# GTEC-UDC/roskfpos

Measured on AMD Instinct MI355X. Metric: EKF predict+update steps/s at 65536 tags x 8 anchors; RMS pos err vs CPU ref, higher is better.
Workload: dtype f64 arithmetic; f64 state and covariance, f32/int32 measurements in HBM (KFPOS_STORE_MIXED)

## Files before the change

__graft_entry__.py:

```python
from __future__ import annotations

import os
import shutil
import subprocess
import sys

ROOT = os.path.dirname(os.path.abspath(__file__))
CSRC = os.path.join(ROOT, "roskfpos_amd", "csrc")
HIP_LIB = os.path.join(CSRC, "libkfpos_hip.so")
ADAPTOR_DEMO = os.path.join(CSRC, "kfpos_replay")


def _stale(target, sources):
    if not os.path.exists(target):
        return True
    mt = os.path.getmtime(target)
    return any(os.path.getmtime(s) > mt for s in sources if os.path.exists(s))


def build(force: bool = False) -> None:
    jobs = str(min(8, os.cpu_count() or 1))
    res = subprocess.run(["make", "-s", "-j", jobs, "-C", CSRC] + (["-B"] if force else []) + ["all"],
                         capture_output=True, text=True)
    if res.returncode != 0:
        sys.stderr.write(res.stdout + res.stderr)
        raise subprocess.CalledProcessError(res.returncode, res.args)
    res = subprocess.run(["make", "-s", "-C", CSRC, "check"], capture_output=True, text=True)
    if res.returncode != 0:
        sys.stderr.write(res.stdout + res.stderr)
        if os.path.exists(HIP_LIB):
            os.remove(HIP_LIB)
        raise RuntimeError("a build-time performance rule is broken (scratch inside a loop / a kernel lost its second "
                           "wavefront per SIMD / the 9-state epoch loop waits for a memory operation just issued / a trip of its gain "
                           "iteration touches memory or branches too often): " + (res.stdout + res.stderr).strip())
    subprocess.check_call(["make", "-s", "-C", os.path.join(ROOT, "oracle")] + (["-B"] if force else []))
    import glob
    core_headers = sorted(glob.glob(os.path.join(CSRC, "kfpos_core*.h"))) + [os.path.join(CSRC, "kfpos_p48.h")]
    emu_dir = os.path.join(ROOT, "tests", "emu")
    emu_so = os.path.join(emu_dir, "libkfpos_emu.so")
    if force or _stale(emu_so, [os.path.join(emu_dir, "kfpos_emu.cpp")] + core_headers):
        subprocess.check_call(["g++", "-O2", "-std=c++17", "-fPIC", "-shared", "-Wno-unknown-pragmas",
                               "-o", emu_so, os.path.join(emu_dir, "kfpos_emu.cpp")])
    fake_dir = os.path.join(ROOT, "tests", "fake_rccl")
    fake_so = os.path.join(fake_dir, "libfake_rccl.so")
    if force or _stale(fake_so, [os.path.join(fake_dir, "fake_rccl.cpp")]):
        subprocess.check_call([shutil.which("hipcc") or "/opt/rocm/bin/hipcc", "-O2", "-std=c++17", "-shared", "-fPIC",
                               "-o", fake_so, os.path.join(fake_dir, "fake_rccl.cpp"), "-lrt"])
    if ROOT not in sys.path:
        sys.path.insert(0, ROOT)
    import roskfpos_amd
    from roskfpos_amd import capi
    capi.load()


def smoke() -> None:
    if ROOT not in sys.path:
        sys.path.insert(0, ROOT)
    sys.path.insert(0, os.path.join(ROOT, "oracle"))
    import numpy as np
    from roskfpos_amd import capi
    from roskfpos_amd.synth import Workload
    import oracle_py

    T, A, S = 256, 8, 12
    w = Workload(T, A)
    for model in (capi.MODEL_TOA, capi.MODEL_TOA_IMU):
        bank = capi.KfposBank(model, T, w.anchors, init_pos=w.init_positions())
        orc = oracle_py.OracleBank(model, T, w.anchors, init_pos=w.init_positions(), n_threads=4)
        err, cov = w.err_est(), w.accel_cov()
        for s in range(S):
            r, a, dt = w.ranges_mm(s), w.accel(s), w.dt_of(s)
            if model == capi.MODEL_TOA_IMU:
                bank.step_toa_imu(r, err, a, cov, dt)
                orc.step_imu(a, cov, 0.0)
                orc.step_toa(r, err, dt)
            else:
                bank.step_toa(r, err, dt)
                orc.step_toa(r, err, dt)
        x, _, _ = bank.get_state()
        xo, _ = orc.get_state()
        rms = float(np.sqrt(((x[:, :3] - xo[:, :3]) ** 2).sum(1).mean()))
        print(f"smoke model={model}: RMS position difference vs oracle = {rms:.3e} m")
        assert rms <= 1e-6, rms
        bank.close()


if __name__ == "__main__":
    build()
    if len(sys.argv) > 1 and sys.argv[1] == "smoke":
        smoke()
```

roskfpos_amd/csrc/kfpos_core_imu9.h:

```cpp
#ifndef KFPOS_CORE_IMU9_H
#define KFPOS_CORE_IMU9_H

namespace kfpos {

constexpr double INFO_FORM_MIN_PIVOT = 1e-7;

struct Tag9 {
    double pos[3], vel[3];
    Cov<9, true> P;
};
struct Imu {
    bool has;
    double acc[3];
    double *ci;
    int ci_stride;
    KFPOS_HD double Wi(int k) const { return ci[(6 + k) * ci_stride]; }
};

KFPOS_FN void imu_whitener(const double s[9], double *ci, int ci_stride) {
    double c00, c11, c22, i00, i11, i22;
    kf_sqrt_rsqrt(s[0], c00, i00);
    const double c10 = s[3] * i00, c20 = s[6] * i00;
    kf_sqrt_rsqrt(s[4] - c10 * c10, c11, i11);
    const double c21 = (s[7] - c20 * c10) * i11;
    kf_sqrt_rsqrt(s[8] - c20 * c20 - c21 * c21, c22, i22);
    const double i10 = -c10 * i00 * i11;
    const double i21 = -c21 * i11 * i22;
    const double i20 = -(c20 * i00 + c21 * i10) * i22;
    ci[0] = i00; ci[ci_stride] = i10; ci[2 * ci_stride] = i20; ci[3 * ci_stride] = i11; ci[4 * ci_stride] = i21;
    ci[5 * ci_stride] = i22;
    double *wi = ci + 6 * ci_stride;
    wi[0] = i00 * i00 + i10 * i10 + i20 * i20;
    wi[ci_stride] = i10 * i11 + i20 * i21;
    wi[2 * ci_stride] = i20 * i22;
    wi[3 * ci_stride] = i11 * i11 + i21 * i21;
    wi[4 * ci_stride] = i21 * i22;
    wi[5 * ci_stride] = i22 * i22;
}

KFPOS_FN void predict9(Cov<9, true> &P, double t, double jolt) {
    const double c = t * t / 2;
    KFPOS_UNROLL
    for (int i = 0; i < 3; ++i) {
        KFPOS_UNROLL
        for (int j = i; j < 3; ++j) {
            const double xpp = P(i, j) + t * P(3 + i, j) + c * P(6 + i, j);
            const double xpv = P(i, 3 + j) + t * P(3 + i, 3 + j) + c * P(6 + i, 3 + j);
            const double xpa = P(i, 6 + j) + t * P(3 + i, 6 + j) + c * P(6 + i, 6 + j);
            P(i, j) = xpp + t * xpv + c * xpa;
        }
    }
    KFPOS_UNROLL
    for (int i = 0; i < 3; ++i) {
        KFPOS_UNROLL
        for (int j = 0; j < 3; ++j) {
            const double xpv = P(i, 3 + j) + t * P(3 + i, 3 + j) + c * P(6 + i, 3 + j);
            const double xpa = P(i, 6 + j) + t * P(3 + i, 6 + j) + c * P(6 + i, 6 + j);
            P(i, 3 + j) = xpv + t * xpa;
        }
    }
    KFPOS_UNROLL
    for (int i = 0; i < 3; ++i) {
        KFPOS_UNROLL
        for (int j = 0; j < 3; ++j) P(i, 6 + j) = P(i, 6 + j) + t * P(3 + i, 6 + j) + c * P(6 + i, 6 + j);
    }
    KFPOS_UNROLL
    for (int i = 0; i < 3; ++i) {
        KFPOS_UNROLL
        for (int j = i; j < 3; ++j) {
            const double xvv = P(3 + i, 3 + j) + t * P(6 + i, 3 + j);
            const double xva = P(3 + i, 6 + j) + t * P(6 + i, 6 + j);
            P(3 + i, 3 + j) = xvv + t * xva;
        }
    }
    KFPOS_UNROLL
    for (int i = 0; i < 3; ++i) {
        KFPOS_UNROLL
        for (int j = 0; j < 3; ++j) P(3 + i, 6 + j) = P(3 + i, 6 + j) + t * P(6 + i, 6 + j);
    }
    const double u[3] = {(t * t * t) / 6, (t * t) / 2, t};
    KFPOS_UNROLL
    for (int k = 0; k < 3; ++k) {
        KFPOS_UNROLL
        for (int a = 0; a < 3; ++a) {
            KFPOS_UNROLL
            for (int b = a; b < 3; ++b) P(k + 3 * a, k + 3 * b) += jolt * u[a] * u[b];
        }
    }
}

KFPOS_HD constexpr int e9(int k) { return k < 3 ? k : k + 3; }

struct Factor9 {
    double lr[6], ilr[3];
    double la[6];
};
KFPOS_FN void factor9(const double mr[6], const double acc[3], const Imu &imu, Factor9 &f) {
    chol3_psd(mr, f.lr, f.ilr);
    if (imu.has) {
        const int cs = imu.ci_stride;
        f.la[0] = acc[0] * imu.ci[0]; f.la[1] = acc[0] * imu.ci[cs]; f.la[2] = acc[0] * imu.ci[2 * cs];
        f.la[3] = acc[1] * imu.ci[3 * cs]; f.la[4] = acc[1] * imu.ci[4 * cs];
        f.la[5] = acc[2] * imu.ci[5 * cs];
    } else {
        KFPOS_UNROLL
        for (int k = 0; k < 6; ++k) f.la[k] = 0.0;
    }
}
KFPOS_FN double L9(const Factor9 &f, int k, int l) {
    if (k < 3 && l < 3) {
        if (k < l) return 0.0;
        return f.lr[l == 0 ? k : (l == 1 ? 2 + k : 5)];
    }
    if (k >= 3 && l >= 3) {
        const int i = k - 3, j = l - 3;
        if (i > j) return 0.0;
        return f.la[i == 0 ? j : (i == 1 ? 2 + j : 5)];
    }
    return 0.0;
}

struct Iekf9Out {
    double w[6];
    double mrlast[6], dlast[3];
    double cost;
    int gain_iters, ml_iters;
    uint32_t flags;
};

template <class SC>
KFPOS_FN void iekf9_weights(const double xhat[9], SC &sc, const Params &pr, bool has_ranging, int n_used,
                            Iekf9Out &o) {
    o.flags = (has_ranging && n_used < 4) ? ST_FEW_RANGES : 0u;
    o.ml_iters = 0;
    if (has_ranging) {
        double pml[3] = {xhat[0], xhat[1], xhat[2]}, e_ml;
        set_weights_ml(sc, pr, 0ull);
        o.ml_iters = ml_estimate(pml, sc, pr, 0ull, n_used, e_ml);
        if (ml_covariance_throws(sc, pr, 0ull, n_used, e_ml)) o.flags |= ST_UPDATE_SKIPPED;
        set_weights_iekf(sc, pr, e_ml, 0ull);
    }
}

template <bool DIAG, bool RANGING, class SC>
KFPOS_FN void iekf9(const double xhat[9], const Cov<9, true> &P, SC &sc, const Params &pr,
                    const Imu &imu, int max_steps, double tol, Iekf9Out &o) {
    double p[3] = {xhat[0], xhat[1], xhat[2]}, acc[3] = {xhat[6], xhat[7], xhat[8]};
    double ve[6] = {0, 0, 0, 0, 0, 0};
    double wl[6] = {0, 0, 0, 0, 0, 0};
    double qd = 0.0, cost = 1e20;
    const bool pivot = RANGING && illconditioned(sc, pr, P);
    KFPOS_UNROLL
    for (int k = 0; k < 6; ++k) o.mrlast[k] = 0.0;
    o.dlast[0] = o.dlast[1] = o.dlast[2] = 0.0;
    o.gain_iters = 0;
    for (int iter = 0; iter < max_steps; ++iter) {
        double c = qd, m0 = 0, m1 = 0, m2 = 0, m3 = 0, m4 = 0, m5 = 0, u0 = 0, u1 = 0, u2 = 0;
        if constexpr (RANGING) {
            for_anchors<SC>(pr, [&](int a) {
                const double dx = p[0] - pr.anchors[3 * a], dy = p[1] - pr.anchors[3 * a + 1],
                             dz = p[2] - pr.anchors[3 * a + 2];
                double d, invd;
                kf_sqrt_rsqrt_sweep(dx * dx + dy * dy + dz * dz, d, invd);
                const double w = sc.W(a), y = sc.R(a) - d;
                const double yw = y * w;
                c += y * yw;
                const double gx = dx * invd, gy = dy * invd, gz = dz * invd;
                u0 += gx * yw; u1 += gy * yw; u2 += gz * yw;
                const double wx = w * gx, wy = w * gy, wz = w * gz;
                m0 += wx * gx; m1 += wx * gy; m2 += wx * gz;
                m3 += wy * gy; m4 += wy * gz; m5 += wz * gz;
            });
        }
        const double m[6] = {m0, m1, m2, m3, m4, m5},
                     u[3] = {u0 + (m0 * ve[0] + m1 * ve[1] + m2 * ve[2]), u1 + (m1 * ve[0] + m3 * ve[1] + m4 * ve[2]),
                             u2 + (m2 * ve[0] + m4 * ve[1] + m5 * ve[2])};
        double ua[3] = {0, 0, 0}, ma[3][3] = {{0, 0, 0}, {0, 0, 0}, {0, 0, 0}};
        if (imu.has) {
            const double ya[3] = {imu.acc[0] - acc[0], imu.acc[1] - acc[1], imu.acc[2] - acc[2]};
            const double va[3] = {ya[0] + acc[0] * ve[3], ya[1] + acc[1] * ve[4], ya[2] + acc[2] * ve[5]};
            if constexpr (DIAG) {
                const double wd[3] = {imu.Wi(0), imu.Wi(3), imu.Wi(5)};
                KFPOS_UNROLL
                for (int i = 0; i < 3; ++i) {
                    const double wy = wd[i] * ya[i];
                    c += ya[i] * wy;
                    ua[i] = acc[i] * (wd[i] * va[i]);
                    ma[i][i] = acc[i] * acc[i] * wd[i];
                }
            } else {
                const double wm[3][3] = {{imu.Wi(0), imu.Wi(1), imu.Wi(2)},
                                         {imu.Wi(1), imu.Wi(3), imu.Wi(4)},
                                         {imu.Wi(2), imu.Wi(4), imu.Wi(5)}};
                KFPOS_UNROLL
                for (int i = 0; i < 3; ++i) {
                    const double wy = wm[i][0] * ya[0] + wm[i][1] * ya[1] + wm[i][2] * ya[2];
                    c += ya[i] * wy;
                    ua[i] = acc[i] * (wm[i][0] * va[0] + wm[i][1] * va[1] + wm[i][2] * va[2]);
                    KFPOS_UNROLL
                    for (int j = 0; j < 3; ++j) ma[i][j] = acc[i] * acc[j] * wm[i][j];
                }
            }
        }
        if (rel_change_below(cost, c, tol)) break;
        cost = c;
        KFPOS_UNROLL
        for (int k = 0; k < 6; ++k) o.mrlast[k] = m[k];
        o.dlast[0] = acc[0]; o.dlast[1] = acc[1]; o.dlast[2] = acc[2];

        const double mr[3][3] = {{m[0], m[1], m[2]}, {m[1], m[3], m[4]}, {m[2], m[4], m[5]}};
        double a11[9], a12[3][3], a21[3][3], a22[3][3];
        KFPOS_UNROLL
        for (int i = 0; i < 3; ++i) {
            KFPOS_UNROLL
            for (int j = 0; j < 3; ++j) {
                a11[3 * i + j] = (i == j ? 1.0 : 0.0) + mr[i][0] * P(0, j) + mr[i][1] * P(1, j) + mr[i][2] * P(2, j);
                a12[i][j] = mr[i][0] * P(0, 6 + j) + mr[i][1] * P(1, 6 + j) + mr[i][2] * P(2, 6 + j);
                if constexpr (DIAG) {
                    a21[i][j] = ma[i][i] * P(6 + i, j);
                    a22[i][j] = (i == j ? 1.0 : 0.0) + ma[i][i] * P(6 + i, 6 + j);
                } else {
                    a21[i][j] = ma[i][0] * P(6, j) + ma[i][1] * P(7, j) + ma[i][2] * P(8, j);
                    a22[i][j] = (i == j ? 1.0 : 0.0) + ma[i][0] * P(6, 6 + j) + ma[i][1] * P(7, 6 + j) + ma[i][2] * P(8, 6 + j);
                }
            }
        }
        if (!pivot) {
            double adj[9];
            const double id1 = kf_rcp(gen3_adjugate(a11, adj));
            double xx[3][3], y1[3];
            KFPOS_UNROLL
            for (int i = 0; i < 3; ++i) {
                y1[i] = (adj[3 * i] * u[0] + adj[3 * i + 1] * u[1] + adj[3 * i + 2] * u[2]) * id1;
                KFPOS_UNROLL
                for (int j = 0; j < 3; ++j)
                    xx[i][j] = (adj[3 * i] * a12[0][j] + adj[3 * i + 1] * a12[1][j] + adj[3 * i + 2] * a12[2][j]) * id1;
            }
            double sc9[9], rhs[3];
            KFPOS_UNROLL
            for (int i = 0; i < 3; ++i) {
                rhs[i] = ua[i] - (a21[i][0] * y1[0] + a21[i][1] * y1[1] + a21[i][2] * y1[2]);
                KFPOS_UNROLL
                for (int j = 0; j < 3; ++j)
                    sc9[3 * i + j] = a22[i][j] - (a21[i][0] * xx[0][j] + a21[i][1] * xx[1][j] + a21[i][2] * xx[2][j]);
            }
            const double id2 = kf_rcp(gen3_adjugate(sc9, adj));
            KFPOS_UNROLL
            for (int i = 0; i < 3; ++i)
                wl[3 + i] = (adj[3 * i] * rhs[0] + adj[3 * i + 1] * rhs[1] + adj[3 * i + 2] * rhs[2]) * id2;
            KFPOS_UNROLL
            for (int i = 0; i < 3; ++i) wl[i] = y1[i] - (xx[i][0] * wl[3] + xx[i][1] * wl[4] + xx[i][2] * wl[5]);
        } else {
            double b4[12], x4[12];
            KFPOS_UNROLL
            for (int i = 0; i < 3; ++i) {
                KFPOS_UNROLL
                for (int j = 0; j < 3; ++j) b4[4 * i + j] = a12[i][j];
                b4[4 * i + 3] = u[i];
            }
            gauss_solve<3, 4>(a11, b4, x4);
            double s9[9], r3[3], wa[3];
            KFPOS_UNROLL
            for (int i = 0; i < 3; ++i) {
                r3[i] = ua[i] - (a21[i][0] * x4[3] + a21[i][1] * x4[7] + a21[i][2] * x4[11]);
                KFPOS_UNROLL
                for (int j = 0; j < 3; ++j)
                    s9[3 * i + j] = a22[i][j] - (a21[i][0] * x4[j] + a21[i][1] * x4[4 + j] + a21[i][2] * x4[8 + j]);
            }
            gauss_solve<3, 1>(s9, r3, wa);
            KFPOS_UNROLL
            for (int i = 0; i < 3; ++i) {
                wl[3 + i] = wa[i];
                wl[i] = x4[4 * i + 3] - (x4[4 * i] * wa[0] + x4[4 * i + 1] * wa[1] + x4[4 * i + 2] * wa[2]);
            }
        }
        qd = 0.0;
        KFPOS_UNROLL
        for (int i = 0; i < 6; ++i) {
            double v = 0.0;
            KFPOS_UNROLL
            for (int k = 0; k < 6; ++k) v += P(e9(i), e9(k)) * wl[k];
            ve[i] = v;
            qd += wl[i] * v;
            if (i < 3) p[i] = xhat[i] + v;
            else acc[i - 3] = xhat[3 + i] + v;
        }
        o.gain_iters++;
    }
    KFPOS_UNROLL
    for (int k = 0; k < 6; ++k) o.w[k] = wl[k];
    o.cost = cost;
}

KFPOS_HD constexpr int s6(int i, int j) { return Cov<6, true>::idx(i, j); }

KFPOS_FN bool ldl6(const Cov<6, true> &a, double L[6][6], double id[6], double rel) {
    bool ok = true;
    double d[6];
    KFPOS_UNROLL
    for (int j = 0; j < 6; ++j) {
        double v[6], dj = a(j, j);
        KFPOS_UNROLL
        for (int k = 0; k < j; ++k) { v[k] = L[j][k] * d[k]; dj -= L[j][k] * v[k]; }
        ok = ok && (dj > rel * a(j, j));
        d[j] = dj;
        id[j] = kf_rcp(dj > 0.0 ? dj : 1.0);
        KFPOS_UNROLL
        for (int i = j + 1; i < 6; ++i) {
            double t = a(i, j);
            KFPOS_UNROLL
            for (int k = 0; k < j; ++k) t -= L[i][k] * v[k];
            L[i][j] = t * id[j];
        }
    }
    return ok;
}
KFPOS_FN bool sym6_inverse(const Cov<6, true> &a, double *out, int stride, double rel) {
    double L[6][6], id[6], W[6][6];
    const bool ok = ldl6(a, L, id, rel);
    KFPOS_UNROLL
    for (int j = 0; j < 6; ++j) {
        KFPOS_UNROLL
        for (int i = j + 1; i < 6; ++i) {
            double t = L[i][j];
            KFPOS_UNROLL
            for (int k = j + 1; k < i; ++k) t += L[i][k] * W[k][j];
            W[i][j] = -t;
        }
    }
    KFPOS_UNROLL
    for (int i = 0; i < 6; ++i) {
        KFPOS_UNROLL
        for (int j = i; j < 6; ++j) {
            double t = (i == j ? 1.0 : W[j][i]) * id[j];
            KFPOS_UNROLL
            for (int k = j + 1; k < 6; ++k) t += W[k][i] * W[k][j] * id[k];
            out[s6(i, j) * stride] = t;
        }
    }
    return ok;
}
KFPOS_HD constexpr int s3(int i, int j) { return i <= j ? (i == 0 ? j : (i == 1 ? 2 + j : 5)) : (j == 0 ? i : (j == 1 ? 2 + i : 5)); }
KFPOS_FN void sym6_solve(const Cov<6, true> &K, const double b[6], double x[6]) {
    const double kpp[6] = {K(0, 0), K(0, 1), K(0, 2), K(1, 1), K(1, 2), K(2, 2)};
    double c1[6], c2[6];
    const double id1 = kf_rcp(sym3_cofactors(kpp, c1));
    double X[3][3], y1[3];
    KFPOS_UNROLL
    for (int i = 0; i < 3; ++i) {
        y1[i] = (c1[s3(i, 0)] * b[0] + c1[s3(i, 1)] * b[1] + c1[s3(i, 2)] * b[2]) * id1;
        KFPOS_UNROLL
        for (int j = 0; j < 3; ++j)
            X[i][j] = (c1[s3(i, 0)] * K(0, 3 + j) + c1[s3(i, 1)] * K(1, 3 + j) + c1[s3(i, 2)] * K(2, 3 + j)) * id1;
    }
    double S[6], rhs[3];
    KFPOS_UNROLL
    for (int i = 0; i < 3; ++i) {
        rhs[i] = b[3 + i] - (K(0, 3 + i) * y1[0] + K(1, 3 + i) * y1[1] + K(2, 3 + i) * y1[2]);
        KFPOS_UNROLL
        for (int j = i; j < 3; ++j)
            S[s3(i, j)] = K(3 + i, 3 + j) - (K(0, 3 + i) * X[0][j] + K(1, 3 + i) * X[1][j] + K(2, 3 + i) * X[2][j]);
    }
    const double id2 = kf_rcp(sym3_cofactors(S, c2));
    KFPOS_UNROLL
    for (int i = 0; i < 3; ++i) x[3 + i] = (c2[s3(i, 0)] * rhs[0] + c2[s3(i, 1)] * rhs[1] + c2[s3(i, 2)] * rhs[2]) * id2;
    KFPOS_UNROLL
    for (int i = 0; i < 3; ++i) x[i] = y1[i] - (X[i][0] * x[3] + X[i][1] * x[4] + X[i][2] * x[5]);
}

struct Sweep9 {
    double c, m[6], u[3];
};
struct Iekf9Iter {
    double ve[6];
    double wl[6];
    double qd, cost;
};

KFPOS_FN void iekf9_sweep4(const double p[3], const double *r, const double *w, const double *b, Sweep9 &s) {
    KFPOS_UNROLL
    for (int a = 0; a < 4; ++a) {
        const double dx = p[0] - b[3 * a], dy = p[1] - b[3 * a + 1], dz = p[2] - b[3 * a + 2];
        double d, invd;
        kf_sqrt_rsqrt_sweep(kf_fma(dz, dz, kf_fma(dy, dy, dx * dx)), d, invd);
        const double y = r[a] - d, yw = y * w[a];
        const double gx = dx * invd, gy = dy * invd, gz = dz * invd;
        const double wx = w[a] * gx, wy = w[a] * gy, wz = w[a] * gz;
        if (a == 0) {
            s.c = y * yw;
            s.u[0] = gx * yw; s.u[1] = gy * yw; s.u[2] = gz * yw;
            s.m[0] = wx * gx; s.m[1] = wx * gy; s.m[2] = wx * gz;
            s.m[3] = wy * gy; s.m[4] = wy * gz; s.m[5] = wz * gz;
        } else {
            s.c = kf_fma(y, yw, s.c);
            s.u[0] = kf_fma(gx, yw, s.u[0]); s.u[1] = kf_fma(gy, yw, s.u[1]); s.u[2] = kf_fma(gz, yw, s.u[2]);
            s.m[0] = kf_fma(wx, gx, s.m[0]); s.m[1] = kf_fma(wx, gy, s.m[1]); s.m[2] = kf_fma(wx, gz, s.m[2]);
            s.m[3] = kf_fma(wy, gy, s.m[3]); s.m[4] = kf_fma(wy, gz, s.m[4]); s.m[5] = kf_fma(wz, gz, s.m[5]);
        }
    }
}
KFPOS_FN void sweep9_add(Sweep9 &s, const Sweep9 &t) {
    s.c += t.c;
    KFPOS_UNROLL
    for (int k = 0; k < 6; ++k) s.m[k] += t.m[k];
    KFPOS_UNROLL
    for (int k = 0; k < 3; ++k) s.u[k] += t.u[k];
}

template <bool RANGING, class SC>
KFPOS_FN void iekf9_sweep(const double p[3], const SC &sc, const Params &pr, Sweep9 &s) {
    if constexpr (!RANGING) {
        s.c = 0.0;
        KFPOS_UNROLL
        for (int k = 0; k < 6; ++k) s.m[k] = 0.0;
        s.u[0] = s.u[1] = s.u[2] = 0.0;
    } else if constexpr (SC::NA == 8 && SC::CHUNK == 0 && !SC::COOP) {
        Sweep9 t;
        iekf9_sweep4(p, &sc.r[0], &sc.w[0], &pr.anchors[0], s);
        iekf9_sweep4(p, &sc.r[4], &sc.w[4], &pr.anchors[12], t);
        sweep9_add(s, t);
    } else {
        double c = 0, m0 = 0, m1 = 0, m2 = 0, m3 = 0, m4 = 0, m5 = 0, u0 = 0, u1 = 0, u2 = 0;
        for_anchors<SC>(pr, [&](int a) {
            const double dx = p[0] - pr.anchors[3 * a], dy = p[1] - pr.anchors[3 * a + 1],
                         dz = p[2] - pr.anchors[3 * a + 2];
            double d, invd;
            kf_sqrt_rsqrt_sweep(dx * dx + dy * dy + dz * dz, d, invd);
            const double w = sc.W(a), y = sc.R(a) - d;
            const double yw = y * w;
            c += y * yw;
            const double gx = dx * invd, gy = dy * invd, gz = dz * invd;
            u0 += gx * yw; u1 += gy * yw; u2 += gz * yw;
            const double wx = w * gx, wy = w * gy, wz = w * gz;
            m0 += wx * gx; m1 += wx * gy; m2 += wx * gz;
            m3 += wy * gy; m4 += wy * gz; m5 += wz * gz;
        });
        s.c = c;
        s.m[0] = m0; s.m[1] = m1; s.m[2] = m2; s.m[3] = m3; s.m[4] = m4; s.m[5] = m5;
        s.u[0] = u0; s.u[1] = u1; s.u[2] = u2;
    }
}

KFPOS_FN void iekf9_spread_reads() {
#if defined(__HIP_DEVICE_COMPILE__)
    KFPOS_UNROLL
    for (int k = 0; k < 20; ++k) {
        __builtin_amdgcn_sched_group_barrier(0x100, 1, 0);
        __builtin_amdgcn_sched_group_barrier(0x002, 10, 0);
    }
#endif
}
struct Iekf9Parked {
    double binv[21], wi[6];
};
template <bool EVERY_TRIP, bool DIAG, bool PIN = !EVERY_TRIP>
KFPOS_FN void iekf9_fetch(const double *binv, int binv_stride, const Imu &imu, Iekf9Parked &pk) {
    const int z = EVERY_TRIP ? kf_opaque_zero() : 0;
    KFPOS_UNROLL
    for (int k = 0; k < 21; ++k) pk.binv[k] = binv[k * binv_stride + z];
    KFPOS_UNROLL
    for (int k = 0; k < 6; ++k) pk.wi[k] = imu.ci[(6 + k) * imu.ci_stride + z];
    if constexpr (PIN) {
        KFPOS_UNROLL
        for (int k = 0; k < 6; ++k) {
            if (!DIAG || k == 0 || k == 3 || k == 5) kf_pin(pk.wi[k]);
        }
    }
}
template <bool DIAG, bool ALLIMU>
KFPOS_FN bool iekf9_pass(const double xhat[9], const Iekf9Parked &pk, const Imu &imu, double tol,
                         const Sweep9 &sw, Iekf9Iter &it, Iekf9Out &o) {
    const double *ve = it.ve;
    const double acc[3] = {xhat[6] + ve[3], xhat[7] + ve[4], xhat[8] + ve[5]};
    double c = it.qd + sw.c;
    const double m0 = sw.m[0], m1 = sw.m[1], m2 = sw.m[2], m3 = sw.m[3], m4 = sw.m[4], m5 = sw.m[5];
    const double m[6] = {m0, m1, m2, m3, m4, m5};
    double u[6] = {sw.u[0] + (m0 * ve[0] + m1 * ve[1] + m2 * ve[2]), sw.u[1] + (m1 * ve[0] + m3 * ve[1] + m4 * ve[2]),
                   sw.u[2] + (m2 * ve[0] + m4 * ve[1] + m5 * ve[2]), 0.0, 0.0, 0.0};
    double ma[6] = {0, 0, 0, 0, 0, 0};
    if (ALLIMU || imu.has) {
        const double ya[3] = {imu.acc[0] - acc[0], imu.acc[1] - acc[1], imu.acc[2] - acc[2]};
        const double va[3] = {ya[0] + acc[0] * ve[3], ya[1] + acc[1] * ve[4], ya[2] + acc[2] * ve[5]};
        if constexpr (DIAG) {
            const double wd[3] = {pk.wi[0], pk.wi[3], pk.wi[5]};
            KFPOS_UNROLL
            for (int i = 0; i < 3; ++i) {
                const double wy = wd[i] * ya[i];
                c += ya[i] * wy;
                u[3 + i] = acc[i] * (wd[i] * va[i]);
            }
            ma[0] = acc[0] * acc[0] * wd[0]; ma[3] = acc[1] * acc[1] * wd[1]; ma[5] = acc[2] * acc[2] * wd[2];
        } else {
            const double wm[3][3] = {{pk.wi[0], pk.wi[1], pk.wi[2]},
                                     {pk.wi[1], pk.wi[3], pk.wi[4]},
                                     {pk.wi[2], pk.wi[4], pk.wi[5]}};
            KFPOS_UNROLL
            for (int i = 0; i < 3; ++i) {
                const double wy = wm[i][0] * ya[0] + wm[i][1] * ya[1] + wm[i][2] * ya[2];
                c += ya[i] * wy;
                u[3 + i] = acc[i] * (wm[i][0] * va[0] + wm[i][1] * va[1] + wm[i][2] * va[2]);
            }
            ma[0] = acc[0] * acc[0] * wm[0][0]; ma[1] = acc[0] * acc[1] * wm[0][1]; ma[2] = acc[0] * acc[2] * wm[0][2];
            ma[3] = acc[1] * acc[1] * wm[1][1]; ma[4] = acc[1] * acc[2] * wm[1][2]; ma[5] = acc[2] * acc[2] * wm[2][2];
        }
    }
    const bool go = !rel_change_below_voted(it.cost, c, tol);
    if (go) {
#ifdef KFPOS_EMU_ITER_TRACE
        kfpos_emu_iter_trace(o.gain_iters, ve, c);
#endif
        it.cost = c;
        KFPOS_UNROLL
        for (int k = 0; k < 6; ++k) o.mrlast[k] = m[k];
        o.dlast[0] = acc[0]; o.dlast[1] = acc[1]; o.dlast[2] = acc[2];

        Cov<6, true> K;
        KFPOS_UNROLL
        for (int k = 0; k < 21; ++k) K.a[k] = pk.binv[k];
        K(0, 0) += m[0]; K(0, 1) += m[1]; K(0, 2) += m[2]; K(1, 1) += m[3]; K(1, 2) += m[4]; K(2, 2) += m[5];
        K(3, 3) += ma[0]; K(4, 4) += ma[3]; K(5, 5) += ma[5];
        if constexpr (!DIAG) { K(3, 4) += ma[1]; K(3, 5) += ma[2]; K(4, 5) += ma[4]; }
        double v[6];
        sym6_solve(K, u, v);
        double *wl = it.wl;
        wl[0] = u[0] - (m[0] * v[0] + m[1] * v[1] + m[2] * v[2]);
        wl[1] = u[1] - (m[1] * v[0] + m[3] * v[1] + m[4] * v[2]);
        wl[2] = u[2] - (m[2] * v[0] + m[4] * v[1] + m[5] * v[2]);
        wl[3] = u[3] - (ma[0] * v[3] + ma[1] * v[4] + ma[2] * v[5]);
        wl[4] = u[4] - (ma[1] * v[3] + ma[3] * v[4] + ma[4] * v[5]);
        wl[5] = u[5] - (ma[2] * v[3] + ma[4] * v[4] + ma[5] * v[5]);
        double qd = 0.0;
        KFPOS_UNROLL
        for (int i = 0; i < 6; ++i) qd += wl[i] * v[i];
        it.qd = qd;
        KFPOS_UNROLL
        for (int i = 0; i < 6; ++i) it.ve[i] = v[i];
        o.gain_iters++;
    }
    return go;
}

#if defined(__HIP_DEVICE_COMPILE__)
KFPOS_FN double lane_pull(double v, int src4) {
    const int lo = __builtin_amdgcn_ds_bpermute(src4, __double2loint(v));
    const int hi = __builtin_amdgcn_ds_bpermute(src4, __double2hiint(v));
    return __hiloint2double(hi, lo);
}
KFPOS_FN int nth_set_bit(uint64_t m, int n) {
    uint32_t w = (uint32_t)m;
    int base = 0;
    const int c0 = __popc(w);
    if (n >= c0) { n -= c0; w = (uint32_t)(m >> 32); base = 32; }
    KFPOS_UNROLL
    for (int width = 16; width >= 1; width >>= 1) {
        const uint32_t low = w & ((1u << width) - 1u);
        const int c = __popc(low);
        if (n >= c) { n -= c; w >>= width; base += width; }
        else w = low;
    }
    return base;
}

template <bool DIAG, bool ACC0>
KFPOS_FN void iekf9_pairs(uint64_t m, const double xhat[9], const double *binv, int binv_stride,
                          const RegScratch<8> &sc, const double *anchor_tab, const Imu &imu, int max_steps, double tol,
                          Iekf9Iter &it, Iekf9Out &o) {
    const int lane = (int)__builtin_amdgcn_mbcnt_hi(~0u, __builtin_amdgcn_mbcnt_lo(~0u, 0u));
    const int g = lane >> 1, h = lane & 1;
    const int n_surv = __popcll(m);
    bool act = g < n_surv;
    const int src = nth_set_bit(m, act ? g : 0);
    const int src4 = src << 2;
    double xh[9];
    KFPOS_UNROLL
    for (int k = 0; k < 3; ++k) {
        xh[k] = lane_pull(xhat[k], src4);
        xh[3 + k] = 0.0;
        xh[6 + k] = ACC0 ? 0.0 : lane_pull(xhat[6 + k], src4);
    }
    Iekf9Iter ct;
    KFPOS_UNROLL
    for (int k = 0; k < 6; ++k) { ct.ve[k] = lane_pull(it.ve[k], src4); ct.wl[k] = lane_pull(it.wl[k], src4); }
    ct.qd = lane_pull(it.qd, src4);
    ct.cost = lane_pull(it.cost, src4);
    Iekf9Out co;
    KFPOS_UNROLL
    for (int k = 0; k < 6; ++k) co.mrlast[k] = lane_pull(o.mrlast[k], src4);
    KFPOS_UNROLL
    for (int k = 0; k < 3; ++k) co.dlast[k] = lane_pull(o.dlast[k], src4);
    co.gain_iters = __builtin_amdgcn_ds_bpermute(src4, o.gain_iters);
    Imu ci;
    ci.has = __builtin_amdgcn_ds_bpermute(src4, imu.has ? 1 : 0) != 0;
    KFPOS_UNROLL
    for (int k = 0; k < 3; ++k) ci.acc[k] = lane_pull(imu.acc[k], src4);
    ci.ci = imu.ci + (src - lane);
    ci.ci_stride = imu.ci_stride;
    double r4[4], w4[4];
    KFPOS_UNROLL
    for (int k = 0; k < 4; ++k) {
        const double r0 = lane_pull(sc.r[k], src4), r1 = lane_pull(sc.r[4 + k], src4);
        const double w0 = lane_pull(sc.w[k], src4), w1 = lane_pull(sc.w[4 + k], src4);
        r4[k] = h ? r1 : r0;
        w4[k] = h ? w1 : w0;
    }
    const double *cbinv = binv + (src - lane);
    const double *b4 = anchor_tab + 12 * h;
    const double b0[3] = {b4[0], b4[1], b4[2]};
    while (act) {
        double bb[12];
        const int z = kf_opaque_zero();
        bb[0] = b0[0]; bb[1] = b0[1]; bb[2] = b0[2];
        KFPOS_UNROLL
        for (int k = 3; k < 12; ++k) bb[k] = b4[k + z];
        Iekf9Parked pk;
        iekf9_fetch<true, DIAG>(cbinv, binv_stride, ci, pk);
        const double p[3] = {xh[0] + ct.ve[0], xh[1] + ct.ve[1], xh[2] + ct.ve[2]};
        Sweep9 sw, other;
        iekf9_sweep4(p, r4, w4, bb, sw);
        other.c = dpp_exchange(sw.c, 0);
        KFPOS_UNROLL
        for (int k = 0; k < 6; ++k) other.m[k] = dpp_exchange(sw.m[k], 0);
        KFPOS_UNROLL
        for (int k = 0; k < 3; ++k) other.u[k] = dpp_exchange(sw.u[k], 0);
        sweep9_add(sw, other);
        iekf9_spread_reads();
        const bool more = iekf9_pass<DIAG, false>(xh, pk, ci, tol, sw, ct, co);
        act = more && co.gain_iters < max_steps;
    }
    const bool owner = (m >> lane) & 1ull;
    const int rank = __popcll(m & ((1ull << lane) - 1ull));
    const int from4 = (owner ? 2 * rank : lane) << 2;
    KFPOS_UNROLL
    for (int k = 0; k < 6; ++k) {
        const double a = lane_pull(ct.wl[k], from4), b = lane_pull(co.mrlast[k], from4);
        if (owner) { it.wl[k] = a; o.mrlast[k] = b; }
    }
    KFPOS_UNROLL
    for (int k = 0; k < 3; ++k) {
        const double a = lane_pull(co.dlast[k], from4);
        if (owner) o.dlast[k] = a;
    }
    const double cst = lane_pull(ct.cost, from4);
    const int gi = __builtin_amdgcn_ds_bpermute(from4, co.gain_iters);
    if (owner) { it.cost = cst; o.gain_iters = gi; }
}
#endif

template <bool DIAG, bool ALLIMU, bool RANGING, bool ACC0 = false, bool HOLD = true, class SC>
KFPOS_FN void iekf9_info(const double xhat[9], const double *binv, int binv_stride, SC &sc, const Params &pr,
                         const Imu &imu, int max_steps, double tol, Iekf9Out &o) {
    Iekf9Iter it;
    KFPOS_UNROLL
    for (int k = 0; k < 6; ++k) { it.ve[k] = 0.0; it.wl[k] = 0.0; o.mrlast[k] = 0.0; }
    it.qd = 0.0;
    it.cost = 1e20;
    o.dlast[0] = o.dlast[1] = o.dlast[2] = 0.0;
    o.gain_iters = 0;
#if defined(__HIP_DEVICE_COMPILE__)
    constexpr bool PAIRS = RANGING && SC::NA == 8 && SC::CHUNK == 0 && !SC::COOP;
    const bool pairs = PAIRS && pr.pair_anchor_tab && __builtin_amdgcn_ballot_w64(true) == ~0ull;
#endif
    bool more = true;
    int stop = max_steps;
#if defined(__HIP_DEVICE_COMPILE__)
    if (pairs) stop = 8 < max_steps ? 8 : max_steps;
#endif
    Iekf9Parked pk;
    if constexpr (HOLD) iekf9_fetch<false, DIAG, true>(binv, binv_stride, imu, pk);
    for (;;) {
        while (more && o.gain_iters < stop) {
            if constexpr (!HOLD) iekf9_fetch<false, DIAG, false>(binv, binv_stride, imu, pk);
            const double p[3] = {xhat[0] + it.ve[0], xhat[1] + it.ve[1], xhat[2] + it.ve[2]};
            Sweep9 sw;
            iekf9_sweep<RANGING>(p, sc, pr, sw);
            more = iekf9_pass<DIAG, ALLIMU>(xhat, pk, imu, tol, sw, it, o);
        }
#if defined(__HIP_DEVICE_COMPILE__)
        if constexpr (PAIRS) {
            if (pairs) {
                const uint64_t m = __builtin_amdgcn_ballot_w64(more && o.gain_iters < max_steps);
                if (m == 0) break;
                if (__popcll(m) <= 32) {
                    iekf9_pairs<DIAG, ACC0>(m, xhat, binv, binv_stride, sc, pr.pair_anchor_tab, imu, max_steps, tol, it, o);
                    break;
                }
                stop = stop + 4 < max_steps ? stop + 4 : max_steps;
                continue;
            }
        }
#endif
        break;
    }
    KFPOS_UNROLL
    for (int k = 0; k < 6; ++k) o.w[k] = it.wl[k];
    o.cost = it.cost;
}

KFPOS_FN void cov_update9(Cov<9, true> &P, const double mr[6], const double d[3], const Imu &imu) {
    Factor9 f;
    factor9(mr, d, imu, f);
    KFPOS_UNROLL
    for (int k = 0; k < 6; ++k) {
        double pt[9], s = 1.0;
        KFPOS_UNROLL
        for (int i = 0; i < 9; ++i) {
            double v = 0.0;
            KFPOS_UNROLL
            for (int l = 0; l < 6; ++l) {
                const bool nz = (l < 3 && k < 3 && l >= k) || (l >= 3 && k >= 3 && l <= k);
                if (nz) v += P(i, e9(l)) * L9(f, l, k);
            }
            pt[i] = v;
        }
        KFPOS_UNROLL
        for (int l = 0; l < 6; ++l) {
            const bool nz = (l < 3 && k < 3 && l >= k) || (l >= 3 && k >= 3 && l <= k);
            if (nz) s += L9(f, l, k) * pt[e9(l)];
        }
        const double is = kf_rcp(s);
        KFPOS_UNROLL
        for (int i = 0; i < 9; ++i) {
            const double pi = pt[i] * is;
            KFPOS_UNROLL
            for (int j = i; j < 9; ++j) P(i, j) -= pi * pt[j];
        }
    }
}

struct CovPark9 {
    double *a;
    int stride;
};

template <bool RANGING, bool HOLD = true, class SC>
KFPOS_FN bool step_imu9_state(Tag9 &tg, SC &sc, const Params &pr, double dt, const Imu &imu, const CovPark9 &park,
                              bool fast, Iekf9Out &o, uint32_t &status) {
    constexpr bool has_ranging = RANGING;
    const int n_valid = has_ranging ? count_used(sc, pr, 0) : 0;
    if (!pr.use_init_pos && (isnan(tg.pos[0]) || isnan(tg.pos[1]))) {
        status = 0;
        if (!has_ranging) return false;
        status = ST_FEW_RANGES;
        if (n_valid < 4) return false;
        double p[3] = {1.0, 1.0, 4.0}, sse, c[6];
        set_weights_ml(sc, pr, 0ull);
        const int it = ml_estimate(p, sc, pr, 0, n_valid, sse);
        status = ST_UPDATE_SKIPPED;
        if (ml_covariance_throws(sc, pr, 0, n_valid, sse)) return false;
        if (!ml_covariance(p, sc, pr, sse, c)) return false;
        tg.pos[0] = p[0]; tg.pos[1] = p[1]; tg.pos[2] = p[2];
        tg.P(0, 0) = c[0]; tg.P(0, 1) = c[1]; tg.P(1, 1) = c[3];
        status = pack_status(ST_ML_INIT, 0, it, -1);
        return false;
    }
    const double c = dt * dt / 2;
    double xhat[9];
    KFPOS_UNROLL
    for (int k = 0; k < 3; ++k) {
        xhat[k] = tg.pos[k] + dt * tg.vel[k] + c * 0.0;
        xhat[3 + k] = tg.vel[k] + dt * 0.0;
        xhat[6 + k] = 0.0;
    }
    predict9(tg.P, dt, pr.jolt);
    Cov<6, true> B;
    KFPOS_UNROLL
    for (int i = 0; i < 6; ++i) {
        KFPOS_UNROLL
        for (int j = i; j < 6; ++j) B(i, j) = tg.P(e9(i), e9(j));
    }
    KFPOS_UNROLL
    for (int k = 0; k < 45; ++k) park.a[k * park.stride] = tg.P.a[k];
    double *binv = park.a + 45 * park.stride;
    const bool invertible = sym6_inverse(B, binv, park.stride, INFO_FORM_MIN_PIVOT);
    iekf9_weights(xhat, sc, pr, has_ranging, n_valid, o);
    if (o.flags & ST_UPDATE_SKIPPED) {
        KFPOS_UNROLL
        for (int k = 0; k < 45; ++k) tg.P.a[k] = park.a[k * park.stride];
        status = ST_UPDATE_SKIPPED;
        return false;
    }
    if (invertible) {
        if (fast) iekf9_info<true, true, RANGING, true, HOLD>(xhat, binv, park.stride, sc, pr, imu, 20, 1e-4, o);
        else iekf9_info<false, false, RANGING, true, HOLD>(xhat, binv, park.stride, sc, pr, imu, 20, 1e-4, o);
        KFPOS_UNROLL
        for (int k = 0; k < 45; ++k) tg.P.a[k] = park.a[k * park.stride];
    } else {
        KFPOS_UNROLL
        for (int k = 0; k < 45; ++k) tg.P.a[k] = park.a[k * park.stride];
        if (fast) iekf9<true, RANGING>(xhat, tg.P, sc, pr, imu, 20, 1e-4, o);
        else iekf9<false, RANGING>(xhat, tg.P, sc, pr, imu, 20, 1e-4, o);
    }
    KFPOS_UNROLL
    for (int i = 0; i < 6; ++i) {
        double v = 0.0;
        KFPOS_UNROLL
        for (int k = 0; k < 6; ++k) v += tg.P(i, e9(k)) * o.w[k];
        if (i < 3) tg.pos[i] = xhat[i] + v;
        else tg.vel[i - 3] = xhat[i] + v;
    }
    status = 0;
    return true;
}
KFPOS_FN uint32_t step_imu9_cov(Tag9 &tg, const Iekf9Out &o, const Imu &imu) {
    cov_update9(tg.P, o.mrlast, o.dlast, imu);
    return pack_status(o.flags, o.gain_iters, o.ml_iters, -1);
}
template <bool RANGING, class SC>
KFPOS_FN uint32_t step_imu9(Tag9 &tg, SC &sc, const Params &pr, double dt, const Imu &imu, const CovPark9 &park) {
    Iekf9Out o;
    uint32_t status;
    if (!step_imu9_state<RANGING>(tg, sc, pr, dt, imu, park, false, o, status)) return status;
    return step_imu9_cov(tg, o, imu);
}

KFPOS_FN void pose9(const Tag9 &tg, double t, double jolt, double pos[3], double vel[3], double cov[9]) {
    const double c = t * t / 2, t3 = (t * t * t) / 6;
    KFPOS_UNROLL
    for (int i = 0; i < 3; ++i) {
        pos[i] = tg.pos[i] + t * tg.vel[i];
        vel[i] = tg.vel[i];
        KFPOS_UNROLL
        for (int j = 0; j < 3; ++j) {
            const Cov<9, true> &P = tg.P;
            const double xpp = P(i, j) + t * P(3 + i, j) + c * P(6 + i, j);
            const double xpv = P(i, 3 + j) + t * P(3 + i, 3 + j) + c * P(6 + i, 3 + j);
            const double xpa = P(i, 6 + j) + t * P(3 + i, 6 + j) + c * P(6 + i, 6 + j);
            cov[3 * i + j] = xpp + t * xpv + c * xpa + (i == j ? jolt * t3 * t3 : 0.0);
        }
    }
}

}
#endif
```

roskfpos_amd/csrc/kfpos_k_imu9.hip:

```cpp
#include "kfpos_kernels.h"

namespace {

template <typename REAL, typename MREAL, int AS, bool RANGING = true>
__global__ __launch_bounds__(WAVE) void k_step_imu9(const KArgs a) {
    extern __shared__ double lds[];
    const int lane = threadIdx.x;
    const size_t t = (size_t)blockIdx.x * WAVE + lane;
    if (t >= (size_t)a.T) return;
    const size_t T = a.T;
    const uint32_t t32 = (uint32_t)t;
    Params pr = make_params(a);
    constexpr bool has_ranging = RANGING;
    constexpr bool AHEAD = sizeof(MREAL) == 4 && !std::is_same<REAL, float>::value;
    const bool fresh_imu = a.mode != MODE_TOA;
    constexpr int NA = AS > 0 ? AS : 1;
    double dt_tag = a.dt_shared;
    if (a.n_steps == 1 && a.dt) {
        dt_tag = a.dt[t32];
        if (dt_tag < 0.0) {
            skipped_lane(a, t, true);
            return;
        }
    }

    uint32_t fl = a.flags[t32];
    RawEpoch<MREAL, NA> raw;
    RawImu<MREAL> rawi;
    if constexpr (AS > 0) {
        if (has_ranging) fetch_epoch<MREAL, AS>(a, t, 0, raw);
    }
    Tag9 tg;
#pragma unroll
    for (int k = 0; k < 3; ++k) {
        tg.pos[k] = (a.pos + k * T)[t32];
        tg.vel[k] = (a.vel + k * T)[t32];
    }
    const CovPark9 park{lds + ((AS == 0 && has_ranging) ? 3 * (size_t)a.A * WAVE : 0) + lane, WAVE};
    Imu imu;
    imu.has = false;
    imu.ci = park.a + 66 * WAVE;
    imu.ci_stride = WAVE;
    if constexpr (AS == 8 && RANGING) {
        if (a.pair9) {
            double *tab = lds + 78 * WAVE;
#pragma unroll
            for (int k = 0; k < 24; ++k) tab[k] = a.anchors[k];
            pr.pair_anchor_tab = tab;
        }
    }
    double cv[9] = {1, 0, 0, 0, 1, 0, 0, 0, 1};
    MREAL rawc[9];
    if (fresh_imu) {
        fetch_imu<MREAL>(a, t, 0, rawi);
        fetch_imu_cov<MREAL>(a, t, 0, rawc);
    } else if (fl & FL_HAS_IMU) {
        imu.has = true;
#pragma unroll
        for (int k = 0; k < 3; ++k) imu.acc[k] = ldrow<MREAL>(a.imu_acc, k, T, t32);
        cv[0] = ldrow<MREAL>(a.imu_cov, 0, T, t32);
        cv[3] = ldrow<MREAL>(a.imu_cov, 1, T, t32);
        cv[4] = ldrow<MREAL>(a.imu_cov, 2, T, t32);
        cv[6] = ldrow<MREAL>(a.imu_cov, 3, T, t32);
        cv[7] = ldrow<MREAL>(a.imu_cov, 4, T, t32);
        cv[8] = ldrow<MREAL>(a.imu_cov, 5, T, t32);
    }
#pragma unroll
    for (int k = 0; k < 45; ++k) tg.P.a[k] = ldcov<REAL>(a.P, k, 45, T, t32);
    if (fresh_imu) {
        imu.has = true;
#pragma unroll
        for (int k = 0; k < 9; ++k) cv[k] = (double)rawc[k];
        if (a.latch) latch_imu_cov<MREAL>(a, T, t32, cv);
    }
    if (imu.has) imu_whitener(cv, imu.ci, imu.ci_stride);
    bool diag = false;
    if (a.imu9_diag) {
        const bool mine = !imu.has || (imu.Wi(1) == 0.0 && imu.Wi(2) == 0.0 && imu.Wi(4) == 0.0);
        diag = __builtin_amdgcn_ballot_w64(mine) == __builtin_amdgcn_ballot_w64(true);
    }
    const bool fast = imu9_fast(diag, imu.has);

    const bool multi = a.n_steps > 1;
    double dt_next = multi ? a.dt_steps[0] : dt_tag;
    constexpr bool IMU_WITH_EPOCH = AHEAD && AS > 0 && RANGING;

    __builtin_amdgcn_s_waitcnt(0x0F70);
    uint32_t s = 0;
    for (int e = 0; e < a.n_steps; ++e) {
        const double dt = dt_next;
        if (multi && e + 1 < a.n_steps) dt_next = a.dt_steps[opaque_uniform(e + 1)];
        if (fresh_imu) {
#pragma unroll
            for (int k = 0; k < 3; ++k) imu.acc[k] = (double)rawi.acc[k];
            if constexpr (AHEAD && !IMU_WITH_EPOCH) {
                if (e + 1 < a.n_steps) fetch_imu<MREAL>(a, opaque_lane(t), opaque_uniform(e + 1), rawi);
            }
        }
        Iekf9Out o;
        auto finish = [&](bool update) {
            if (a.traj) {
#pragma unroll
                for (int k = 0; k < 3; ++k) (a.traj + ((size_t)opaque_uniform(e) * 3 + k) * T)[t32] = tg.pos[k];
            }
            if (update) s = step_imu9_cov(tg, o, imu);
        };
        if constexpr (AS > 0) {
            RegScratch<AS> sc;
            if (has_ranging) {
                unpack_epoch<MREAL, AS>(raw, sc);
                if (e + 1 < a.n_steps) {
                    if constexpr (AHEAD) {
                        fetch_epoch<MREAL, AS>(a, opaque_lane(t), opaque_uniform(e + 1), raw);
                        if constexpr (IMU_WITH_EPOCH) {
                            if (fresh_imu) fetch_imu<MREAL>(a, opaque_lane(t), opaque_uniform(e + 1), rawi);
                        }
                    }
                }
            } else {
#pragma unroll
                for (int k = 0; k < AS; ++k) sc.r[k] = sc.e[k] = sc.w[k] = 0.0;
            }
            finish(step_imu9_state<RANGING>(tg, sc, pr, dt, imu, park, fast, o, s));
            if constexpr (!AHEAD) {
                if (e + 1 < a.n_steps) {
                    if (fresh_imu) fetch_imu<MREAL>(a, opaque_lane(t), opaque_uniform(e + 1), rawi);
                    if (has_ranging) fetch_epoch<MREAL, AS>(a, opaque_lane(t), opaque_uniform(e + 1), raw);
                }
            }
        } else {
            Scratch sc{nullptr, nullptr, nullptr, WAVE};
            if (has_ranging) sc = stage_epoch_lds<MREAL>(a, lds, lane, t, opaque_uniform(e));
            finish(step_imu9_state<RANGING>(tg, sc, pr, dt, imu, park, fast, o, s));
            if constexpr (!AHEAD) {
                if (e + 1 < a.n_steps && fresh_imu) fetch_imu<MREAL>(a, opaque_lane(t), opaque_uniform(e + 1), rawi);
            }
        }
        if constexpr (cov_is_rounded<REAL>()) {
            if (e + 1 < a.n_steps) {
#pragma unroll
                for (int k = 0; k < 45; ++k) tg.P.a[k] = round_cov<REAL>(tg.P.a[k]);
            }
        }
    }

    if (fresh_imu && a.latch) {
#pragma unroll
        for (int k = 0; k < 3; ++k) strow<MREAL>(a.imu_acc, k, T, t32, imu.acc[k]);
        fl |= FL_HAS_IMU;
    }
    bool fin = true;
#pragma unroll
    for (int k = 0; k < 3; ++k) {
        (a.pos + k * T)[t32] = tg.pos[k];
        (a.vel + k * T)[t32] = tg.vel[k];
        fin &= isfinite(tg.pos[k]) & isfinite(tg.vel[k]);
    }
#pragma unroll
    for (int k = 0; k < 45; ++k) {
        stcov<REAL>(a.P, k, 45, T, t32, tg.P.a[k]);
        fin &= isfinite(tg.P.a[k]);
    }
    const bool waiting = !a.use_init_pos && isnan(tg.pos[0]);
    if (!fin && !waiting) s |= ST_NONFINITE;
    a.flags[t32] = fl | FL_STARTED;
    if (a.status) a.status[t32] = s;
}

}

template <typename REAL, typename MREAL>
static kfpos_k::step_kernel_t imu9_of(int as, bool ranging) {
    if (!ranging) return k_step_imu9<REAL, MREAL, 0, false>;
    if (as == 8) return k_step_imu9<REAL, MREAL, 8>;
    return k_step_imu9<REAL, MREAL, 0>;
}
kfpos_k::step_kernel_t kfpos_k::imu9_kernel(int st, int as, bool ranging) {
    return KFPOS_BY_STORAGE(st, imu9_of, as, ranging);
}
```

Baseline: 2.119 billion.

## Rotate IMU9 epoch loop so covariance predict and park run ahead of the update

```diff
diff --git a/__graft_entry__.py b/__graft_entry__.py
--- a/__graft_entry__.py
+++ b/__graft_entry__.py
@@ -32,7 +32,8 @@
             os.remove(HIP_LIB)
         raise RuntimeError("a build-time performance rule is broken (scratch inside a loop / a kernel lost its second "
                            "wavefront per SIMD / the 9-state epoch loop waits for a memory operation just issued / a trip of its gain "
-                           "iteration touches memory or branches too often): " + (res.stdout + res.stderr).strip())
+                           "iteration touches memory or branches too often / its epoch loop carries a covariance across the back-edge in "
+                           "registers): " + (res.stdout + res.stderr).strip())
     subprocess.check_call(["make", "-s", "-C", os.path.join(ROOT, "oracle")] + (["-B"] if force else []))
     import glob
     core_headers = sorted(glob.glob(os.path.join(CSRC, "kfpos_core*.h"))) + [os.path.join(CSRC, "kfpos_p48.h")]
diff --git a/roskfpos_amd/csrc/kfpos_core_imu9.h b/roskfpos_amd/csrc/kfpos_core_imu9.h
--- a/roskfpos_amd/csrc/kfpos_core_imu9.h
+++ b/roskfpos_amd/csrc/kfpos_core_imu9.h
@@ -646,7 +646,7 @@
 }
 #endif
 
-template <bool DIAG, bool ALLIMU, bool RANGING, bool ACC0 = false, bool HOLD = true, class SC>
+template <bool DIAG, bool ALLIMU, bool RANGING, bool ACC0 = false, bool HOLD = true, bool SETTLE = false, class SC>
 KFPOS_FN void iekf9_info(const double xhat[9], const double *binv, int binv_stride, SC &sc, const Params &pr,
                          const Imu &imu, int max_steps, double tol, Iekf9Out &o) {
     Iekf9Iter it;
@@ -667,6 +667,9 @@
 #endif
     Iekf9Parked pk;
     if constexpr (HOLD) iekf9_fetch<false, DIAG, true>(binv, binv_stride, imu, pk);
+#if defined(__HIP_DEVICE_COMPILE__)
+    if constexpr (HOLD && SETTLE) __builtin_amdgcn_s_waitcnt(0xC07F);
+#endif
     for (;;) {
         while (more && o.gain_iters < stop) {
             if constexpr (!HOLD) iekf9_fetch<false, DIAG, false>(binv, binv_stride, imu, pk);
@@ -731,6 +734,76 @@
     double *a;
     int stride;
 };
+
+KFPOS_FN bool imu9_started(const Tag9 &tg, const Params &pr) {
+    return pr.use_init_pos || !(isnan(tg.pos[0]) || isnan(tg.pos[1]));
+}
+template <bool RANGING, class SC>
+KFPOS_FN bool imu9_ml_init(double pos[3], SC &sc, const Params &pr, int n_valid, double c[6], uint32_t &status) {
+    status = 0;
+    if (!RANGING) return false;
+    status = ST_FEW_RANGES;
+    if (n_valid < 4) return false;
+    double p[3] = {1.0, 1.0, 4.0}, sse;
+    set_weights_ml(sc, pr, 0ull);
+    const int it = ml_estimate(p, sc, pr, 0, n_valid, sse);
+    status = ST_UPDATE_SKIPPED;
+    if (ml_covariance_throws(sc, pr, 0, n_valid, sse)) return false;
+    if (!ml_covariance(p, sc, pr, sse, c)) return false;
+    pos[0] = p[0]; pos[1] = p[1]; pos[2] = p[2];
+    status = pack_status(ST_ML_INIT, 0, it, -1);
+    return true;
+}
+KFPOS_FN void imu9_predict_state(const Tag9 &tg, double dt, double xhat[9]) {
+    const double c = dt * dt / 2;
+    KFPOS_UNROLL
+    for (int k = 0; k < 3; ++k) {
+        xhat[k] = tg.pos[k] + dt * tg.vel[k] + c * 0.0;
+        xhat[3 + k] = tg.vel[k] + dt * 0.0;
+        xhat[6 + k] = 0.0;
+    }
+}
+KFPOS_FN void imu9_park(const Cov<9, true> &P, const CovPark9 &park) {
+    KFPOS_UNROLL
+    for (int k = 0; k < 45; ++k) park.a[k * park.stride] = P.a[k];
+}
+KFPOS_FN void imu9_unpark(Cov<9, true> &P, const CovPark9 &park) {
+    KFPOS_UNROLL
+    for (int k = 0; k < 45; ++k) P.a[k] = park.a[k * park.stride];
+}
+KFPOS_FN bool imu9_predict_park(Cov<9, true> &P, double dt, double jolt, const CovPark9 &park) {
+    predict9(P, dt, jolt);
+    Cov<6, true> B;
+    KFPOS_UNROLL
+    for (int i = 0; i < 6; ++i) {
+        KFPOS_UNROLL
+        for (int j = i; j < 6; ++j) B(i, j) = P(e9(i), e9(j));
+    }
+    imu9_park(P, park);
+    return sym6_inverse(B, park.a + 45 * park.stride, park.stride, INFO_FORM_MIN_PIVOT);
+}
+template <bool RANGING, bool HOLD, bool SETTLE, class SC>
+KFPOS_FN void imu9_iterate(Tag9 &tg, const double xhat[9], SC &sc, const Params &pr, const Imu &imu,
+                           const CovPark9 &park, bool fast, bool invertible, Iekf9Out &o) {
+    double *binv = park.a + 45 * park.stride;
+    if (invertible) {
+        if (fast) iekf9_info<true, true, RANGING, true, HOLD, SETTLE>(xhat, binv, park.stride, sc, pr, imu, 20, 1e-4, o);
+        else iekf9_info<false, false, RANGING, true, HOLD, SETTLE>(xhat, binv, park.stride, sc, pr, imu, 20, 1e-4, o);
+        imu9_unpark(tg.P, park);
+    } else {
+        imu9_unpark(tg.P, park);
+        if (fast) iekf9<true, RANGING>(xhat, tg.P, sc, pr, imu, 20, 1e-4, o);
+        else iekf9<false, RANGING>(xhat, tg.P, sc, pr, imu, 20, 1e-4, o);
+    }
+    KFPOS_UNROLL
+    for (int i = 0; i < 6; ++i) {
+        double v = 0.0;
+        KFPOS_UNROLL
+        for (int k = 0; k < 6; ++k) v += tg.P(i, e9(k)) * o.w[k];
+        if (i < 3) tg.pos[i] = xhat[i] + v;
+        else tg.vel[i - 3] = xhat[i] + v;
+    }
+}
 
 template <bool RANGING, bool HOLD = true, class SC>
 KFPOS_FN bool step_imu9_state(Tag9 &tg, SC &sc, const Params &pr, double dt, const Imu &imu, const CovPark9 &park,
@@ -801,6 +874,38 @@
     status = 0;
     return true;
 }
+KFPOS_FN bool step_imu9_head(Tag9 &tg, const Params &pr, double dt, const CovPark9 &park) {
+    if (imu9_started(tg, pr)) return imu9_predict_park(tg.P, dt, pr.jolt, park);
+    imu9_park(tg.P, park);
+    return false;
+}
+template <bool RANGING, bool HOLD = true, class SC>
+KFPOS_FN bool step_imu9_state_parked(Tag9 &tg, SC &sc, const Params &pr, double dt, const Imu &imu,
+                                     const CovPark9 &park, bool fast, bool invertible, Iekf9Out &o, uint32_t &status) {
+    constexpr bool has_ranging = RANGING;
+    const int n_valid = has_ranging ? count_used(sc, pr, 0) : 0;
+    if (!imu9_started(tg, pr)) {
+        double c[6];
+        if (imu9_ml_init<RANGING>(tg.pos, sc, pr, n_valid, c, status)) {
+            park.a[Cov<9, true>::idx(0, 0) * park.stride] = c[0];
+            park.a[Cov<9, true>::idx(0, 1) * park.stride] = c[1];
+            park.a[Cov<9, true>::idx(1, 1) * park.stride] = c[3];
+        }
+        imu9_unpark(tg.P, park);
+        return false;
+    }
+    double xhat[9];
+    imu9_predict_state(tg, dt, xhat);
+    iekf9_weights(xhat, sc, pr, has_ranging, n_valid, o);
+    if (o.flags & ST_UPDATE_SKIPPED) {
+        imu9_unpark(tg.P, park);
+        status = ST_UPDATE_SKIPPED;
+        return false;
+    }
+    imu9_iterate<RANGING, HOLD, true>(tg, xhat, sc, pr, imu, park, fast, invertible, o);
+    status = 0;
+    return true;
+}
 KFPOS_FN uint32_t step_imu9_cov(Tag9 &tg, const Iekf9Out &o, const Imu &imu) {
     cov_update9(tg.P, o.mrlast, o.dlast, imu);
     return pack_status(o.flags, o.gain_iters, o.ml_iters, -1);
diff --git a/roskfpos_amd/csrc/kfpos_k_imu9.hip b/roskfpos_amd/csrc/kfpos_k_imu9.hip
--- a/roskfpos_amd/csrc/kfpos_k_imu9.hip
+++ b/roskfpos_amd/csrc/kfpos_k_imu9.hip
@@ -1,6 +1,14 @@
 #include "kfpos_kernels.h"
 
 namespace {
+
+template <typename W>
+__device__ inline void in_agpr(W &w) {
+    static_assert(sizeof(W) == 4, "one register");
+    asm volatile("" : "+a"(w));
+}
+
+__device__ inline void forget(double &v) { asm volatile("" : "=v"(v)); }
 
 template <typename REAL, typename MREAL, int AS, bool RANGING = true>
 __global__ __launch_bounds__(WAVE) void k_step_imu9(const KArgs a) {
@@ -84,9 +92,58 @@
     const bool multi = a.n_steps > 1;
     double dt_next = multi ? a.dt_steps[0] : dt_tag;
     constexpr bool IMU_WITH_EPOCH = AHEAD && AS > 0 && RANGING;
+    constexpr bool ROTATE = IMU_WITH_EPOCH && AS == 8 && std::is_same<REAL, double>::value;
 
     __builtin_amdgcn_s_waitcnt(0x0F70);
     uint32_t s = 0;
+    if constexpr (ROTATE) {
+        bool invertible = step_imu9_head(tg, pr, dt_next, park);
+        double latched[3] = {0.0, 0.0, 0.0};
+        if (!fresh_imu && imu.has) {
+#pragma unroll
+            for (int k = 0; k < 3; ++k) latched[k] = imu.acc[k];
+        }
+        for (int e = 0; e < a.n_steps; ++e) {
+            const double dt = dt_next;
+            const bool more = e + 1 < a.n_steps;
+            if (multi && more) dt_next = a.dt_steps[opaque_uniform(e + 1)];
+#pragma unroll
+            for (int k = 0; k < NA; ++k) { in_agpr(raw.mm[k]); in_agpr(raw.e[k]); }
+            if (fresh_imu) {
+#pragma unroll
+                for (int k = 0; k < 3; ++k) in_agpr(rawi.acc[k]);
+            }
+#pragma unroll
+            for (int k = 0; k < 3; ++k) imu.acc[k] = fresh_imu ? (double)rawi.acc[k] : latched[k];
+            RegScratch<NA> sc;
+            unpack_epoch<MREAL, NA>(raw, sc);
+#pragma unroll
+            for (int k = 0; k < NA; ++k) { kfpos::kf_pin(sc.r[k]); kfpos::kf_pin(sc.e[k]); }
+#pragma unroll
+            for (int k = 0; k < 3; ++k) kfpos::kf_pin(imu.acc[k]);
+            asm volatile("" ::: "memory");
+            const int ahead = opaque_uniform(more ? e + 1 : e);
+            fetch_epoch<MREAL, NA>(a, opaque_lane(t), ahead, raw);
+            if (fresh_imu) fetch_imu<MREAL>(a, opaque_lane(t), ahead, rawi);
+            Iekf9Out o;
+#pragma unroll
+            for (int k = 0; k < 6; ++k) { forget(o.w[k]); forget(o.mrlast[k]); }
+#pragma unroll
+            for (int k = 0; k < 3; ++k) forget(o.dlast[k]);
+            const bool update = step_imu9_state_parked<RANGING>(tg, sc, pr, dt, imu, park, fast, invertible, o, s);
+            if (a.traj) {
+#pragma unroll
+                for (int k = 0; k < 3; ++k) (a.traj + ((size_t)opaque_uniform(e) * 3 + k) * T)[t32] = tg.pos[k];
+            }
+            if (update) s = step_imu9_cov(tg, o, imu);
+            if (more) {
+                static_assert(!cov_is_rounded<REAL>(), "a rounded covariance is rounded here, in front of the head");
+                invertible = step_imu9_head(tg, pr, dt_next, park);
+#pragma unroll
+                for (int k = 0; k < 45; ++k) forget(tg.P.a[k]);
+            }
+        }
+    } else
     for (int e = 0; e < a.n_steps; ++e) {
         const double dt = dt_next;
         if (multi && e + 1 < a.n_steps) dt_next = a.dt_steps[opaque_uniform(e + 1)];
```

Result: faster. 2.158 billion (median of 6 runs) (+1.8%).
